# dsilvestro/npBNN

Hardware: AMD Instinct MI355X
Metric: MCMC iterations/sec (full fwd+lik per proposal) (higher is better)
Workload: dtype f16x3-split/f32

## Files before the change

### include/npbnn_hip.h

```cpp
#ifndef NPBNN_HIP_H
#define NPBNN_HIP_H

#include <stddef.h>
#include <stdint.h>

#ifdef __cplusplus
extern "C" {
#endif

#define NPBNN_ABI_VERSION 1
#define NPBNN_MAX_LAYERS 8
#define NPBNN_MAX_WIDTH 4096
#define NPBNN_MAX_TARGETS 16
#define NPBNN_XSTATE_DOUBLES (4 + NPBNN_MAX_TARGETS)

enum {
    NPBNN_OK = 0,
    NPBNN_E_ARG = -1,
    NPBNN_E_STATE = -2,
    NPBNN_E_HIP = -3,
    NPBNN_E_NOMEM = -4,
    NPBNN_E_COMM = -5,
    NPBNN_E_RANGE = -6,
    NPBNN_E_SYNC = -7,
// ... 130 lines not shown
    int32_t slope_term_in_prior;
} npbnn_chain_cfg;
#define NPBNN_SCHED_AUTO 0
#define NPBNN_SCHED_SERIAL 1
#define NPBNN_SCHED_OVERLAP 2
#define NPBNN_SCHED_OVERLAP2 3

#define NPBNN_SCHED_PERSIST 4

#define NPBNN_SCHED_PERSIST_SERIAL 5

typedef struct {
    double loglik, logprior;
    double sigma[NPBNN_MAX_TARGETS];
    int64_t n_accepted;
    int32_t n_passes;
    int32_t n_candidates;
    int32_t n_void_passes;
    int32_t schedule;
    double temperature;
    int32_t iterations_done;
    int32_t overflow;
    double slopes[NPBNN_MAX_LAYERS];
} npbnn_chain_result;

int npbnn_chain_run(npbnn_ctx* ctx, const npbnn_chain_cfg* cfg, double* W_inout, const double* mask_packed,
                    int32_t K, int32_t M, const int32_t* idx, const double* delta, const int32_t* cnt,
                    const double* log_u, uint8_t* out_accepted, double* out_loglik_prop, double* out_logprior_prop,
                    npbnn_chain_result* result);

enum { NPBNN_PROP_NORMAL = 0, NPBNN_PROP_UNIFORM = 1, NPBNN_PROP_FIXED_NORMAL = 2, NPBNN_PROP_NORMAL_NORMALIZED = 3 };
typedef struct {
    int32_t proposal_kind;
    int32_t M;
    const int32_t* idx;
    const double* val;
    const int32_t* cnt;
    const int32_t* h_idx;
    const double* h_val;
    const double* h_fac;
    const int32_t* h_cnt;
    const int32_t* layer_mask;
    double* ind_inout;
    const int32_t* ind_ptr;
    const int32_t* ind_pos;
    double prior_ind1;
// ... 76 lines not shown
```

### npbnn_amd/_capi.py

```python
import ctypes as C
import os

import numpy as np

MAX_LAYERS = 8
MAX_WIDTH = 4096
MAX_TARGETS = 16
XSTATE_DOUBLES = 4 + MAX_TARGETS

ACT_RELU, ACT_LEAKY, ACT_SWISH, ACT_TANH = 0, 1, 2, 3
OUT_SOFTMAX, OUT_IDENTITY, OUT_SOFTPLUS_HALF = 0, 1, 2
(LIK_CATEGORICAL, LIK_GAUSS, LIK_GAUSS_PRED_SIGMA, LIK_POISSON, LIK_NEGBIN, LIK_NEGBIN2D,
 LIK_NEGBIN_BASE10, LIK_NONE) = range(8)
PRIOR_UNIFORM, PRIOR_NORMAL, PRIOR_CAUCHY, PRIOR_LAPLACE = 0, 1, 2, 3
TRAIN, TEST = 0, 1
OPT_L0_PRECISION = 1
OPT_FAST_TAILS = 2
OPT_PERSISTENT = 3
OPT_TRAINABLE_SLOPES = 4
OPT_WIDE = 5
L0_AUTO, L0_F32, L0_F16 = 0, 1, 2
INFO_L0_F16, INFO_WAVES_PER_BLOCK, INFO_N_CU, INFO_FAST_TAILS, INFO_TURN_NS_OVERLAPPED, INFO_TURN_NS_BETWEEN, INFO_MAX_CANDIDATES = 1, 2, 3, 4, 5, 6, 7
INFO_IT_NS_OVERLAPPED, INFO_IT_NS_BETWEEN = 8, 9
INFO_WIDE = 10
# ... 32 lines not shown


class EvalOut(C.Structure):
    _fields_ = [("loglik", C.c_double), ("sigma", C.c_double * MAX_TARGETS),
                ("sum_r", C.c_double * MAX_TARGETS), ("sum_r2", C.c_double * MAX_TARGETS),
                ("n_rows", C.c_int64)]


class ChainCfg(C.Structure):
    _fields_ = [("prior_kind", C.c_int32), ("prior_scale", C.c_double * MAX_LAYERS), ("w_bound", C.c_double),
                ("temperature", C.c_double), ("lik_temp", C.c_double), ("sigma_given", C.c_int32),
                ("sigma", C.c_double * MAX_TARGETS), ("cur_loglik", C.c_double), ("cur_logprior", C.c_double),
                ("cur_sigma", C.c_double * MAX_TARGETS), ("force_f32", C.c_int32), ("n_candidates", C.c_int32),
                ("schedule", C.c_int32), ("reserved_", C.c_int32), ("sigma_mult", C.POINTER(C.c_double)),
                ("hastings", C.POINTER(C.c_double)), ("prior_scale_w", C.POINTER(C.c_double)),
                ("slope_idx", C.POINTER(C.c_int32)), ("slope_delta", C.POINTER(C.c_double)),
                ("cur_slopes", C.c_double * MAX_LAYERS), ("n_slopes", C.c_int32), ("slope_term_in_prior", C.c_int32)]


class ChainResult(C.Structure):
    _fields_ = [("loglik", C.c_double), ("logprior", C.c_double), ("sigma", C.c_double * MAX_TARGETS),
                ("n_accepted", C.c_int64), ("n_passes", C.c_int32), ("n_candidates", C.c_int32),
                ("n_void_passes", C.c_int32), ("schedule", C.c_int32), ("temperature", C.c_double),
                ("iterations_done", C.c_int32), ("overflow", C.c_int32), ("slopes", C.c_double * MAX_LAYERS)]


class GeneralCfg(C.Structure):
    _fields_ = [("proposal_kind", C.c_int32), ("M", C.c_int32), ("idx", C.POINTER(C.c_int32)), ("val", C.POINTER(C.c_double)),
                ("cnt", C.POINTER(C.c_int32)), ("h_idx", C.POINTER(C.c_int32)), ("h_val", C.POINTER(C.c_double)),
                ("h_fac", C.POINTER(C.c_double)), ("h_cnt", C.POINTER(C.c_int32)), ("layer_mask", C.POINTER(C.c_int32)),
                ("ind_inout", C.POINTER(C.c_double)), ("ind_ptr", C.POINTER(C.c_int32)), ("ind_pos", C.POINTER(C.c_int32)),
                ("prior_ind1", C.c_double), ("has_indicator_prior", C.c_int32), ("reserved_", C.c_int32),
                ("find_inout", C.POINTER(C.c_double)), ("feature_means", C.POINTER(C.c_double)),
                ("find_ptr", C.POINTER(C.c_int32)), ("find_pos", C.POINTER(C.c_int32)), ("find_use", C.POINTER(C.c_int32))]


PROP_NORMAL, PROP_UNIFORM, PROP_FIXED_NORMAL, PROP_NORMAL_NORMALIZED = 0, 1, 2, 3


class ChainJob(C.Structure):
    _fields_ = [("ctx", C.c_void_p), ("cfg", C.POINTER(ChainCfg)), ("W_inout", C.POINTER(C.c_double)),
                ("mask_packed", C.POINTER(C.c_double)), ("M", C.c_int32), ("chain_id", C.c_int32),
                ("idx", C.POINTER(C.c_int32)), ("delta", C.POINTER(C.c_double)), ("cnt", C.POINTER(C.c_int32)),
                ("log_u", C.POINTER(C.c_double)), ("out_accepted", C.POINTER(C.c_uint8)),
                ("out_loglik_prop", C.POINTER(C.c_double)), ("out_logprior_prop", C.POINTER(C.c_double)),
                ("out_state", C.POINTER(C.c_double)), ("out_cold_w", C.POINTER(C.c_double)),
                ("result", C.POINTER(ChainResult))]
# ... 125 lines not shown
```

### npbnn_amd/backend.py

```python
import ctypes as C
import os
from operator import is_ as _is
from time import perf_counter as _now

import numpy as np

from . import _capi as capi


_PACKED_VIEWS = {}


def note_packed_views(layers, base):
    if len(_PACKED_VIEWS) >= 32:
        _PACKED_VIEWS.clear()
    _PACKED_VIEWS[id(layers[0])] = (tuple(layers), base)


def pack_weights(weights):
    first = weights[0]
    known = _PACKED_VIEWS.get(id(first))
    if known is not None and len(known[0]) == len(weights) and all(map(_is, known[0], weights)):
        return known[1].copy()
    base = getattr(first, "base", None)
# ... 444 lines not shown
        k = self.arch.n_targets
        if sigma is not None:
            for j, v in enumerate(np.broadcast_to(sigma, (k,))):
                cfg.sigma[j] = float(v)
        if cur_sigma is not None:
            for j, v in enumerate(np.broadcast_to(cur_sigma, (k,))):
                cfg.cur_sigma[j] = float(v)
        cfg.cur_loglik, cfg.cur_logprior = float(cur_loglik), float(cur_logprior)
        cfg.n_candidates = int(n_candidates)
        cfg.schedule = int(schedule)
        cfg.force_f32 = 0
        if sigma_mult is not None:
            cfg._keep = (capi.as_f64(sigma_mult), capi.as_f64(hastings))
            cfg.sigma_mult, cfg.hastings = capi.dptr(cfg._keep[0]), capi.dptr(cfg._keep[1])
        else:
            cfg._keep = None
            cfg.sigma_mult = cfg.hastings = None

    def _result_dict(self, res):
        k = self.arch.n_targets
        return dict(loglik=res.loglik, logprior=res.logprior, sigma=np.array(res.sigma[:k]) if k else _NO_SIGMA,
                    n_accepted=res.n_accepted, n_passes=res.n_passes, n_candidates=res.n_candidates,
                    n_void_passes=res.n_void_passes, schedule=res.schedule, temperature=res.temperature,
                    iterations_done=res.iterations_done, overflow=res.overflow, slopes=res.slopes)

    def chain_run(self, weights, idx, delta, cnt, log_u, prior_kind, prior_scale, w_bound, temperature, lik_temp,
                  cur_loglik, cur_logprior, cur_sigma=None, sigma=None, mask=None, n_candidates=0, schedule=0, sigma_mult=None,
                  hastings=None, slopes=None, fixed_slopes=None):
        w = pack_weights(weights) if isinstance(weights, (list, tuple)) else capi.as_f64(weights).copy()
        K, M = idx.shape
        cfg = self.__dict__.get("_chain_cfg")
        if cfg is None:
            cfg = self._chain_cfg = capi.ChainCfg()
            self._chain_res = capi.ChainResult()
        self._fill_chain_cfg(cfg, prior_kind, prior_scale, w_bound, temperature, lik_temp, cur_loglik, cur_logprior,
                             cur_sigma, sigma, n_candidates, schedule, sigma_mult, hastings, slopes, fixed_slopes)
        m = None if mask is None else (pack_weights(mask) if isinstance(mask, (list, tuple)) else capi.as_f64(mask))
        if idx.dtype != np.int32 or not idx.flags.c_contiguous:
            idx = np.ascontiguousarray(idx, dtype=np.int32)
        if cnt.dtype != np.int32 or not cnt.flags.c_contiguous:
            cnt = np.ascontiguousarray(cnt, dtype=np.int32)
        delta = capi.as_f64(delta)
        log_u = capi.as_f64(log_u)
        acc = np.empty(K, dtype=np.uint8)
        llp, lpp = np.empty(K), np.empty(K)
        res = self._chain_res
        run = capi.chain_run_by_address(self._lib)
# ... 219 lines not shown
```

### npbnn_amd/csrc/npbnn_chain.hip.h

```cpp
#pragma once
#include "npbnn_common.hip.h"
#include "npbnn_pack.hip.h"

namespace npbnn {

struct FinalizeParams {
    const double* partials;
    int n_waves;
    int lik_kind;
    int k_targets;
    long long n_rows;
    double lik_temp;
    int sigma_given;
    double sigma[NPBNN_MAX_TARGETS];
    npbnn_eval_out* out;
};

__device__ __forceinline__ int partial_value_count(int lik_kind, int k_targets) { return lik_kind == NPBNN_LIK_GAUSS ? 1 + 2 * k_targets : 1; }
__device__ __forceinline__ int partial_value_index(int item, int k_targets) {
    return item <= k_targets ? item : 1 + NPBNN_MAX_TARGETS + (item - k_targets - 1);
}

__device__ __forceinline__ void reduce_partials(const double* __restrict__ partials, int n_blocks, int n_items, int k_targets, double* tot ) {
    const int lane = threadIdx.x & 63, wave = threadIdx.x >> 6, nw = blockDim.x >> 6;
// ... 39 lines not shown
    if (threadIdx.x == 0) loglik_from_totals(tot, f.lik_kind, f.k_targets, f.n_rows, f.lik_temp, f.sigma_given, f.sigma, f.out);
}
#endif

struct ChainDev {
    double logLik, logPrior;
    double sigma[NPBNN_MAX_TARGETS];
    double cand_logPrior[2][kMaxCand];
    int t;
    int n_accepted;
    int n_passes;
    int void_launch;
    int n_void;
    int seg_end;
    double temperature;
    double logPrior_rep;
    int seg_idx;
    int poisoned;
    int prepared;
    int aborted;
    int started;
    int exchanged;
    int done[4];
};

struct SlopeState {
    double cur[kMaxLayers];
    double term;
    double cand[2][kMaxCand][kMaxLayers];
};
__host__ __device__ inline double slope_prior_term(const double* s, int n) {
    double sum = 0.0;
    for (int l = 0; l < n; ++l) sum += s[l];
    return 2.302585092994046 * -sum * 10.0;
}

struct SpecState;
struct ChainParams {
    ChainDev* st;
    PassDesc* pass;
    double* w_cur;
    const double* mask;
    const int* idx;
    const double* delta;
    const int* cnt;
    const double* log_u;
// ... 146 lines not shown
    int out;
    int launch;
};
__device__ __forceinline__ StepPlan overlapped_plan(int launch) {
    StepPlan pl;
    pl.first = 0;
    pl.resum = 0;
    pl.dec = launch >= 1 ? ((launch - 1) & 1) : -1;
    pl.fly = launch & 1;
    pl.out = (launch + 1) & 1;
    pl.launch = launch;
    return pl;
}

struct StepShared {
    double tot[kMaxCand][kPartialStride];
    double red[16];
    double red3[kMaxCand][16];
    npbnn_eval_out o;
    double s_lp;
    int s_accepted, s_t, s_start, s_lim;
};

template <bool WIDE = false>
__device__ __forceinline__ void chain_step(const ChainParams& c_generic, const StepPlan pl, StepShared& sh) {
    typedef const __attribute__((address_space(4))) ChainParams ConstChainParams;
    ConstChainParams& c = *(ConstChainParams*)&c_generic;
    const int tid = threadIdx.x;
    ChainDev* st = c.st;
    const int lik_kind = c.net.lik_kind;
    const size_t pv_stride = (size_t)kMaxCand * c.M;
    const size_t part_stride = (size_t)kMaxCand * kPartialStride * c.n_blocks;
    const int stamp_row = pl.first ? 0 : (c.pass[pl.dec >= 0 ? pl.dec : 0].t0 & 1023);
#define NPBNN_STAMP(k) do { if (c.stamps && threadIdx.x == 0) c.stamps[(size_t)stamp_row * 8 + (k)] = wall_clock64(); } while (0)
    NPBNN_STAMP(0);

    if (pl.resum && c.prior_kind != NPBNN_PRIOR_UNIFORM) {
        double lp = 0.0;
        for (int l = 0; l < c.net.n_layers; ++l) {
            const auto& L = c.net.L[l];
            const int n = L.out_dim * (L.in_dim + L.has_bias);
            const double sc = c.prior_scale[l];
            if (c.prior_scale_w) {
                for (int i = tid; i < n; i += blockDim.x) lp += log_prior_density(c.prior_kind, c.w_cur[L.w_off + i], c.prior_scale_w[L.w_off + i]);
            } else if (c.prior_kind == NPBNN_PRIOR_NORMAL) {
                double q = 0.0;
                for (int i = tid; i < n; i += blockDim.x) { const double w = c.w_cur[L.w_off + i]; q += w * w; }
                lp += -0.5 * q / (sc * sc);
                if (tid == 0) lp -= (double)n * (log(sc) + 0.9189385332046727418);
            } else {
                for (int i = tid; i < n; i += blockDim.x) lp += log_prior_density(c.prior_kind, c.w_cur[L.w_off + i], sc);
            }
        }
        const double s = block_sum(lp, sh.red);
        if (tid == 0) st->logPrior = s;
    }
    if (pl.resum && c.slopes && tid == 0) {
        const double term = c.slope_term_in ? slope_prior_term(c.slopes->cur, c.n_slopes) : 0.0;
        c.slopes->term = term;
        if (c.prior_kind != NPBNN_PRIOR_UNIFORM) st->logPrior += term;
    }

    int t0 = 0, n_pend = 0;
    if (pl.dec >= 0) {
        t0 = c.pass[pl.dec].t0;
        n_pend = c.pass[pl.dec].n_cand;
        if (pl.fly >= 0 && st->void_launch == pl.launch - 1) n_pend = 0;
    }
    double prefetch_sink = 0.0;
    bool deferred = false;
    if constexpr (WIDE) deferred = c.prep_terms != nullptr;
    if (pl.fly < 0 && !deferred) {
        const int r_lo = t0 + (pl.first ? 0 : 1), r_hi = min(c.K, t0 + n_pend + c.D);
        double sink = 0.0;
        for (int r = r_lo; r < r_hi; ++r)
            if (tid < c.M) sink += (double)c.idx[(size_t)r * c.M + tid] + c.delta[(size_t)r * c.M + tid] + (double)c.pos[(size_t)r * c.M + tid];
        prefetch_sink = sink;
    }
    double d_cand[kMaxCand], d_logu[kMaxCand], d_h[kMaxCand], d_ll = 0.0, d_lp = 0.0, d_temp = 1.0;
#pragma unroll
    for (int j = 0; j < kMaxCand; ++j) { d_cand[j] = 0.0; d_logu[j] = 0.0; d_h[j] = 0.0; }
    if constexpr (WIDE) {
        if (deferred && n_pend > 0) {
            constexpr int TS = 3;
            int n_terms[kMaxCand];
            double x[kMaxCand][TS];
#pragma unroll
            for (int j = 0; j < kMaxCand; ++j) {
                n_terms[j] = j < n_pend ? c.pass[pl.dec].cnt[j] : 0;
#pragma unroll
// ... 57 lines not shown
                for (int b = lane + 256; b < c.n_blocks; b += 64) s += src[b];
                s = butterfly_sum_f64(s);
                if (lane == 0) sh.tot[j][v] = s;
            }
        }
        __syncthreads();
        NPBNN_STAMP(2);
        if (tid == 0) {
            int accepted = -1, n_done = n_pend;
#pragma unroll
            for (int j = 0; j < kMaxCand; ++j) {
                if (j < n_pend && accepted < 0) {
                    const int t = t0 + j;
                    if (c.sigma_mult) {
                        double sg[NPBNN_MAX_TARGETS];
                        for (int q = 0; q < c.net.k_targets; ++q) sg[q] = st->sigma[q] * c.sigma_mult[(size_t)t * c.net.k_targets + q];
                        loglik_from_totals(sh.tot[j], lik_kind, c.net.k_targets, c.n_rows, c.lik_temp, 1, sg, &sh.o);
                    } else {
                        loglik_from_totals(sh.tot[j], lik_kind, c.net.k_targets, c.n_rows, c.lik_temp, c.sigma_given, c_generic.sigma_fixed, &sh.o);
                    }
                    const double lp = d_cand[j];
                    const double post_new = sh.o.loglik + lp, post_old = d_ll + d_lp;
                    const int a = ((post_new - post_old) * d_temp + d_h[j] >= d_logu[j]) ? 1 : 0;
                    c.out_acc[t] = (unsigned char)a;
                    c.out_ll[t] = sh.o.loglik;
                    c.out_lp[t] = lp;
                    if (a) {
                        st->logLik = sh.o.loglik;
                        st->logPrior = lp;
                        st->logPrior_rep = lp;
                        st->n_accepted += 1;
                        if (lik_kind == NPBNN_LIK_GAUSS)
                            for (int q = 0; q < c.net.k_targets; ++q) st->sigma[q] = sh.o.sigma[q];
                        if (c.slopes) {
                            for (int l = 0; l < c.n_slopes; ++l) c.slopes->cur[l] = c.slopes->cand[pl.dec][j][l];
                            c.slopes->term = slope_prior_term(c.slopes->cur, c.n_slopes);
                        }
                        accepted = j;
                        n_done = j + 1;
                        sh.s_lp = lp;
                    }
                }
            }
            if (accepted < 0) sh.s_lp = d_lp;
            st->t = t0 + n_done;
            st->n_passes += 1;
            sh.s_accepted = accepted;
            sh.s_t = t0 + n_done;
            int start = t0 + n_done;
            if (pl.fly >= 0) {
                if (accepted >= 0) {
                    __hip_atomic_store(&st->void_launch, pl.launch, __ATOMIC_RELAXED, __HIP_MEMORY_SCOPE_AGENT);
                    if (c.pass[pl.fly].n_cand > 0) st->n_void += 1;
                } else {
                    start = c.pass[pl.fly].t0 + c.pass[pl.fly].n_cand;
                }
            }
            sh.s_start = start;
            sh.s_lim = st->seg_end;
        }
        __syncthreads();
        NPBNN_STAMP(3);
        const int a = sh.s_accepted;
        if constexpr (WIDE) {
            constexpr int CU = 4;
            if (a >= 0) {
                const size_t row = (size_t)(t0 + a) * c.M;
                const int n = c.cnt[t0 + a];
                const double* pv = c.pv + (size_t)pl.dec * pv_stride;
                for (int e0 = tid; e0 < n; e0 += CU * (int)blockDim.x) {
                    int ci[CU], cp[CU];
                    double cv[CU];
                    float cs[CU];
    #pragma unroll
                    for (int u = 0; u < CU; ++u) {
// ... 55 lines not shown

    NPBNN_STAMP(4);
    const int t_new = sh.s_start;
    int n_new = sh.s_lim - t_new;
    if (n_new > c.D) n_new = c.D;
    if (n_new < 0) n_new = 0;
    if (n_new == 0) {
        if (tid == 0) {
            PassDesc d;
            d.t0 = t_new;
            d.n_cand = 0;
            for (int j = 0; j < kMaxCand; ++j) d.cnt[j] = 0;
            d.pad[0] = sh.s_t >= sh.s_lim ? 1 : 0;
            d.pad[1] = d.pad[2] = 0;
            c.pass[pl.out] = d;
        }
        return;
    }
    double dlp[kMaxCand];
    if constexpr (WIDE) {
#pragma unroll
        for (int j = 0; j < kMaxCand; ++j) dlp[j] = 0.0;
    }
    if (!deferred) {
        const double* __restrict__ wcur = c.w_cur;
        const double* __restrict__ mask = c.mask;
        double* __restrict__ pv_out = c.pv + (size_t)pl.out * pv_stride;
        int woff[kMaxLayers];
        double half_inv_s2[kMaxLayers], layer_scale[kMaxLayers];
#pragma unroll
        for (int q = 0; q < kMaxLayers; ++q) {
            woff[q] = q < c.net.n_layers ? c.net.L[q].w_off : 0x7fffffff;
            half_inv_s2[q] = c.half_inv_s2[q];
            layer_scale[q] = c.prior_scale[q];
        }
        constexpr int ES = 2;
        int ii[kMaxCand][ES], pp[kMaxCand][ES], cn[kMaxCand];
        double dd[kMaxCand][ES], bb[kMaxCand][ES], mm[kMaxCand][ES], sw[kMaxCand][ES];
        float ss[kMaxCand][ES];
#pragma unroll
        for (int j = 0; j < kMaxCand; ++j) {
            dlp[j] = 0.0;
            cn[j] = j < n_new ? c.cnt[t_new + j] : 0;
#pragma unroll
            for (int u = 0; u < ES; ++u) {
                const int e = tid + u * (int)blockDim.x;
                ii[j][u] = -1; pp[j][u] = 0; dd[j][u] = 0.0; ss[j][u] = 1.0f;
                if (j < n_new && e < c.M) {
                    const size_t k = (size_t)(t_new + j) * c.M + e;
                    ii[j][u] = c.idx[k];
                    dd[j][u] = c.delta[k];
                    pp[j][u] = c.pos[k];
                    if (c.pscale) ss[j][u] = c.pscale[k];
                }
            }
        }
#pragma unroll
        for (int j = 0; j < kMaxCand; ++j)
#pragma unroll
            for (int u = 0; u < ES; ++u)
                if (!(tid + u * (int)blockDim.x < cn[j])) { ii[j][u] = -1; pp[j][u] = 0; dd[j][u] = 0.0; ss[j][u] = 1.0f; }
#pragma unroll
        for (int j = 0; j < kMaxCand; ++j)
#pragma unroll
            for (int u = 0; u < ES; ++u) {
                const int i = ii[j][u];
// ... 76 lines not shown
        PassDesc d;
        d.t0 = t_new;
        d.n_cand = n_new;
        for (int j = 0; j < kMaxCand; ++j) {
            double sj = 0.0;
            for (int w = 0; w < (int)(blockDim.x >> 6); ++w) sj += sh.red3[j][w];
            if (c.slopes && j < n_new) {
                const int k = c.slope_idx[t_new + j];
                const double step = c.slope_delta[t_new + j];
                double sum = 0.0;
                for (int l = 0; l < kMaxLayers; ++l) {
                    double v = l < c.n_slopes ? c.slopes->cur[l] : 0.0;
                    if (l == k) {
                        v += step;
                        if (v > 1.0) v = 1.0 - (v - 1.0);
                        if (v < 0.0) v = 0.0 + (0.0 - v);
                    }
                    c.slopes->cand[pl.out][j][l] = v;
                    if (l < c.n_slopes) sum += v;
                }
                sj += 2.302585092994046 * -sum * 10.0 - c.slopes->term;
            }
            if (j < n_new) st->cand_logPrior[pl.out][j] = base_lp + sj;
            d.cnt[j] = j < n_new ? c.cnt[t_new + j] : 0;
        }
        d.pad[0] = d.pad[1] = d.pad[2] = 0;
        c.pass[pl.out] = d;
    }
    if (prefetch_sink == 1.2345e300) c.out_lp[0] = prefetch_sink;
    NPBNN_STAMP(6);
#undef NPBNN_STAMP
}

constexpr unsigned long long kSyncTimeoutTicks = 25000000ull;

__device__ __forceinline__ bool sync_wait_ge(ChainDev* st, const int* word, int target, unsigned long long timeout_ticks = kSyncTimeoutTicks) {
    const unsigned long long t0 = wall_clock64();
    while (__hip_atomic_load(word, __ATOMIC_RELAXED, __HIP_MEMORY_SCOPE_AGENT) < target) {
        if (__hip_atomic_load(&st->aborted, __ATOMIC_RELAXED, __HIP_MEMORY_SCOPE_AGENT)) return false;
        if (wall_clock64() - t0 > timeout_ticks) {
            __hip_atomic_store(&st->aborted, 1, __ATOMIC_RELAXED, __HIP_MEMORY_SCOPE_AGENT);
            return false;
        }
        __builtin_amdgcn_s_sleep(2);
    }
    return !__hip_atomic_load(&st->aborted, __ATOMIC_RELAXED, __HIP_MEMORY_SCOPE_AGENT);
}
// ... 631 lines not shown
```

### npbnn_amd/csrc/npbnn_chain_api.hip

```cpp
#define NPBNN_KERNELS_CHAIN
#include "npbnn_ctx.hip.h"

extern "C" int npbnn_comm_allgather_inplace_stream_(npbnn_comm* c, double* d_buf, int count, void* stream);
extern "C" int npbnn_comm_info_(const npbnn_comm* c, int* device, int* rank, int* nranks);
extern "C" void npbnn_comm_abort_(npbnn_comm* c);
extern "C" int npbnn_comm_wait_stream_(npbnn_comm* c, void* stream, const char* what);

namespace {

struct ResLayout { size_t w, cnt, logu, acc, llp, lpp, total; };
ResLayout res_layout(size_t kc, size_t wb) {
    const auto up256 = [](size_t v) { return (v + 255) / 256 * 256; };
    ResLayout L;
    L.w = 512;
    L.cnt = L.w + up256(wb);
    L.logu = L.cnt + up256(kc * sizeof(int));
    L.acc = L.logu + up256(kc * sizeof(double));
    L.llp = L.acc + up256(kc);
    L.lpp = L.llp + up256(kc * sizeof(double));
    L.total = L.lpp + up256(kc * sizeof(double));
    return L;
}

struct ChainBatch {
// ... 215 lines not shown
        HIP_TRY(ctx, hipMemcpyAsync(ctx->d_delta, delta, need * sizeof(double), hipMemcpyHostToDevice, st));
    }
    stage_mark(ctx, "copy of indices + deviates", &t_stage);
    const bool f16 = ctx->net.l0_f16 != 0;
    ChainDev init{};
    init.logLik = cfg->cur_loglik;
    init.logPrior = cfg->cur_logprior;
    init.logPrior_rep = cfg->cur_logprior;
    for (int j = 0; j < NPBNN_MAX_TARGETS; ++j) init.sigma[j] = cfg->cur_sigma[j];
    init.t = 0;
    init.n_accepted = 0;
    init.n_passes = 0;
    init.void_launch = -2;
    init.n_void = 0;
    init.seg_end = (seg_len > 0 && seg_len < K) ? seg_len : K;
    init.temperature = cfg->temperature;
    init.seg_idx = 0;
    init.poisoned = 0;
    init.prepared = -1;
    init.aborted = 0;
    init.started = -1;
    init.exchanged = 0;
    for (int i = 0; i < 4; ++i) init.done[i] = 0;
    {
        memset(ctx->h_res, 0, 512);
        memcpy(ctx->h_res, &init, sizeof(ChainDev));
        memcpy(ctx->h_res + RL.w, W_in, wb);
        memcpy(ctx->h_res + RL.cnt, cnt, (size_t)K * sizeof(int));
        memcpy(ctx->h_res + RL.logu, log_u, (size_t)K * sizeof(double));
        HIP_TRY(ctx, hipMemcpyAsync(ctx->d_res, ctx->h_res, RL.acc, hipMemcpyHostToDevice, st));
    }
    stage_mark(ctx, "copy of state + weights", &t_stage);
    for (int l = 0; l < kMaxLayers; ++l)
        ctx->net.act_prm[l] = (!cfg->slope_idx && l < cfg->n_slopes && l < NPBNN_MAX_LAYERS) ? (float)cfg->cur_slopes[l] : 0.f;
    ChainParams c{};
    c.st = ctx->d_chain;
    c.pass = reinterpret_cast<PassDesc*>(reinterpret_cast<char*>(ctx->d_eparams) + offsetof(EvalParams, pass_desc));
    c.w_cur = ctx->d_wcur;
    c.mask = mask_packed ? ctx->d_mask : nullptr;
    c.idx = ctx->d_idx;
    c.delta = ctx->d_delta;
    c.cnt = ctx->d_cnt;
    c.log_u = ctx->d_logu;
    c.hastings = nullptr;
    c.sigma_mult = nullptr;
    if (cfg->sigma_mult || cfg->hastings) {
// ... 284 lines not shown
    const int overflow = (ctx->net.l0_f16 && (flags & kFlagF16Range)) ? 1 : 0;
    if (overflow && !exchange_run)
        return fail(ctx, NPBNN_E_RANGE, "chain_run: a layer-0 weight left the fp16 range during this batch");
    {
        const char* b = ctx->h_res;
        memcpy(W_inout, b + B.RL.w, B.wb);
        memcpy(out_accepted, b + B.RL.acc, (size_t)k_take);
        if (out_loglik_prop) memcpy(out_loglik_prop, b + B.RL.llp, (size_t)k_take * sizeof(double));
        if (out_logprior_prop) memcpy(out_logprior_prop, b + B.RL.lpp, (size_t)k_take * sizeof(double));
    }
    for (int l = 0; l < NPBNN_MAX_LAYERS; ++l) result->slopes[l] = 0.0;
    if (ctx->batch_slopes) {
        SlopeState fs;
        HIP_TRY(ctx, hipMemcpy(&fs, ctx->d_slopes, sizeof(SlopeState), hipMemcpyDeviceToHost));
        for (int l = 0; l < kMaxLayers && l < NPBNN_MAX_LAYERS; ++l) result->slopes[l] = fs.cur[l];
    }
    result->loglik = fin.logLik;
    result->logprior = fin.n_accepted > 0 ? fin.logPrior_rep : cfg->cur_logprior;
    for (int j = 0; j < NPBNN_MAX_TARGETS; ++j) result->sigma[j] = fin.sigma[j];
    result->n_accepted = fin.n_accepted;
    result->n_passes = fin.n_passes;
    result->n_candidates = B.D;
    result->n_void_passes = fin.n_void;
    result->schedule = B.schedule;
    result->temperature = fin.temperature;
    result->iterations_done = k_take;
    result->overflow = overflow;
    return NPBNN_OK;
}

}

extern "C" {

int npbnn_chain_run(npbnn_ctx* ctx, const npbnn_chain_cfg* cfg, double* W_inout, const double* mask_packed, int32_t K, int32_t M,
                    const int32_t* idx, const double* delta, const int32_t* cnt, const double* log_u, uint8_t* out_accepted,
                    double* out_loglik_prop, double* out_logprior_prop, npbnn_chain_result* result) {
    if (!ctx) return fail(nullptr, NPBNN_E_ARG, "null ctx");
    if (!result || !out_accepted) return fail(ctx, NPBNN_E_ARG, "chain_run: bad arguments");
    static const bool timing = getenv("NPBNN_CHAIN_TIMING") != nullptr;
    ChainBatch B;
    int rc = chain_prepare(ctx, cfg, W_inout, mask_packed, K, M, idx, delta, cnt, log_u, 0, &B);
    if (rc) return rc;
    hipStream_t st = ctx->stream;
    int t_done = 0, n_rounds = 0;
    const ChainDev* now = reinterpret_cast<const ChainDev*>(ctx->h_res.get());
// ... 456 lines not shown
```

### npbnn_amd/csrc/npbnn_eval.hip.h

```cpp
#pragma once
#include "npbnn_common.hip.h"
#include "npbnn_chain.hip.h"

namespace npbnn {

typedef void (*eval_fn_t)(const EvalParams*, int, int);
constexpr int kLikCat = 0, kLikGauss = 1, kLikGen = 2;
__host__ __device__ inline int lik_class(int lik_kind) {
    return lik_needs_row_scratch(lik_kind) ? kLikGen : (lik_kind == NPBNN_LIK_GAUSS ? kLikGauss : kLikCat);
}

template <int LK>
struct TileAcc {
    double ll;
};
template <>
struct TileAcc<kLikGauss> {
    double s1[4], s2[4];
};
constexpr int kFastGaussTargets = 2;

__device__ __forceinline__ int uni(int v) { return __builtin_amdgcn_readfirstlane(v); }
__device__ __forceinline__ float uni(float v) { return __uint_as_float(__builtin_amdgcn_readfirstlane(__float_as_uint(v))); }
__device__ __forceinline__ long long uni(long long v) {
// ... 402 lines not shown
    const int GN = (CHAIN && D > 1) ? uni(p.group_n) : 0;
    const int G = (int)gridDim.x - (GN ? GN : chain ? 1 : 0);
    if (GN && bid >= G) {
        StepShared& sh = *reinterpret_cast<StepShared*>(smem);
        chain_step(*uni(p.group[bid - G].chain), overlapped_plan(launch0), sh);
        return;
    }
    const bool sync = chain && uni(p.sync_mode);
    const int ebid = sync ? bid - 1 : bid;
    const int share_rot = (CHAIN && sync && !GN) ? uni(p.share_rot) : 0;
    int lbid = ebid;
    for (int i = 0; i < launch0 && share_rot > 0; ++i) { lbid += share_rot; if (lbid >= G) lbid -= G; }
    if (chain && bid == (sync ? 0 : G)) {
        StepShared& sh = *reinterpret_cast<StepShared*>(smem);
        int* const lds_flag = reinterpret_cast<int*>(smem + sizeof(StepShared));
        if (SPEC && uni(p.sync_mode) == 3) {
            SpecShared& sp = *reinterpret_cast<SpecShared*>(smem + ((sizeof(StepShared) + 64 + 15) & ~(size_t)15));
            if (chain->mask) spec_rounds<true>(*chain, launch0, launch_end, G, sh, sp, lds_flag);
            else spec_rounds<false>(*chain, launch0, launch_end, G, sh, sp, lds_flag);
            return;
        }
        for (int launch = launch0; launch < launch_end; ++launch) {
            if (sync && !sync_step_enter(*chain, launch, G, lds_flag)) return;
            chain_step(*chain, overlapped_plan(launch), sh);
            if (sync) sync_step_leave(chain->st, launch + 1, next_enqueued && launch + 1 == launch_end);
            if (launch + 1 < launch_end) {
                __syncthreads();
                if (threadIdx.x == 0) {
                    const PassDesc& nx = chain->pass[overlapped_plan(launch).out];
                    *lds_flag = (nx.n_cand == 0 && nx.pad[0] == 1) ? 1 : 0;
                }
                __syncthreads();
                if (*lds_flag) return;
                __syncthreads();
            }
        }
        return;
    }
#ifdef NPBNN_EXP_PROLOGUE_STAMPS
    unsigned long long t_prev_pass0 = 0;
#endif
    constexpr bool LOOK = CHAIN && !SPEC;
    int ahead_t0 = -1;
    int ahead_cnt[D];
#pragma unroll
    for (int j = 0; j < D; ++j) ahead_cnt[j] = 0;
    for (int launch = launch0; launch < launch_end; ++launch, lbid = (lbid + share_rot >= G ? lbid + share_rot - G : lbid + share_rot)) {
// ... 632 lines not shown
                consume();
            }
            if (n_issue < KT0) {
                NPBNN_WAIT_VMCNT(0);
                for (int kt = n_issue; kt < KT0; kt += STEP) consume();
            }
            q += KT0;
        } else {
            for (int kt = 0; kt < KT0; kt += STEP, q += STEP) {
                if (pf_q < Q) {
                    if constexpr (F16) issue_pair();
                    else issue_next();
                }
                wait_younger(pf_q - q - STEP);
                consume();
            }
        }

        if (void_flag) void_seen = __hip_atomic_load(void_flag, __ATOMIC_RELAXED, __HIP_MEMORY_SCOPE_AGENT);
        run_tail(acc0, tseq, tile);
    }
    }
    __builtin_amdgcn_s_waitcnt(0x0f70);
    const int tid_tiles = tid;
    {
    int tid_epi = tid_tiles;
    if constexpr (NPBNN_LAUNDER_TID) {
        tid_epi = threadIdx.x;
        asm volatile("" : "+v"(tid_epi));
    }
    const int tid = tid_epi;
    const int lane = tid & 63;
    const int n = lane & 15, kq = lane >> 4;

    NPBNN_ESTAMP(4);
    if (stamps && lane == 0) stamps[(size_t)gridDim.x * 8 + (size_t)bid * 16 + wave] = wall_clock64();
    const bool look = LOOK && sync && n_loop > 1 && launch + 1 < launch_end && !GN && g_partials != nullptr;
    int* const look_words = reinterpret_cast<int*>(smem + D * IB + (size_t)wpb * uni(p.lay.wave_lds));
    if (g_partials || GN) {
#pragma unroll
        for (int j = 0; j < D; ++j) {
            if constexpr (LK == kLikGauss) {
#pragma unroll
                for (int i = 0; i < GI; ++i) {
                    A[j].s1[i] = row_sum_f64(A[j].s1[i]);
                    A[j].s2[i] = row_sum_f64(A[j].s2[i]);
// ... 17 lines not shown
        }
        double* wsum = reinterpret_cast<double*>(smem + D * IB);
#pragma unroll
        for (int j = 0; j < D; ++j) {
            double* ws = wsum + ((size_t)j * wpb + wave) * kPartialStride;
            if constexpr (LK == kLikGauss) {
                if (lane == 0) ws[0] = 0.0;
                if (n == 0) {
#pragma unroll
                    for (int i = 0; i < 4; ++i) {
                        ws[1 + 4 * kq + i] = i < GI ? A[j].s1[i < GI ? i : 0] : 0.0;
                        ws[1 + NPBNN_MAX_TARGETS + 4 * kq + i] = i < GI ? A[j].s2[i < GI ? i : 0] : 0.0;
                    }
                }
            } else {
                if (lane == 0) ws[0] = A[j].ll;
            }
        }
        if (look && wave == 0 && lane < 8)
            look_words[lane] = nx_ready ? nx_desc : 0;
        asm volatile("" :: "v"(nx_prepared), "v"(nx_desc));
        __syncthreads();
        constexpr int nvals = (LK == kLikGauss) ? kPartialStride : 1;
        for (int item = tid - ((int)blockDim.x - 64); item >= 0 && item < D * nvals; item += 64) {
            const int j = item / nvals, v = item % nvals;
            if constexpr (LK == kLikGauss) { if (v != 0 && ((v - 1) & (NPBNN_MAX_TARGETS - 1)) >= p_generic.net.k_targets) continue; }
            double s = 0.0;
            for (int w = 0; w < wpb; ++w) s += wsum[((size_t)j * wpb + w) * kPartialStride + v];
            double* const dst = GN ? p.group[j].partials + (((size_t)par * kMaxCand) * kPartialStride + v) * G + lbid
                                   : g_partials + (((size_t)par * kMaxCand + j) * kPartialStride + v) * G + lbid;
            if constexpr (SPEC) {
                if (early_copy) { spec_part_store(spec_part + spec_part_index(par, j, v, lbid), s, spec_gen0 + (unsigned)launch + 1u); continue; }
            }
            if (sync) __hip_atomic_store(dst, s, __ATOMIC_RELAXED, __HIP_MEMORY_SCOPE_AGENT);
            else *dst = s;
        }
    }
    NPBNN_ESTAMP(6);
    if (sync) {
        __syncthreads();
        if (threadIdx.x == blockDim.x - 64 && !(SPEC && early_copy)) sync_eval_leave(st_dev, launch);
        if constexpr (LOOK) {
            if (look && look_words[1] > 0) {
                ahead_t0 = uni(look_words[0]);
#pragma unroll
                for (int j = 0; j < D; ++j) ahead_cnt[j] = uni(look_words[2 + (j < kMaxCand ? j : 0)]);
                stage_images();
            }
        }
    }
    }
    NPBNN_ESTAMPX(4);
    }
#undef NPBNN_ESTAMP
}

}
```

### npbnn_amd/sampler.py

```python
import _thread
import functools
import operator
import os
import queue
import threading

import numpy as np

from . import _capi as capi
from .backend import note_packed_views, pack_weights
from .likelihoods import (CalcAccuracy, CalcAccuracyRegression, CalcLabelAccuracy,
                          CalcLabelAccuracyRegression, SkipAccuracy, SkipAccuracyVec, calc_likelihood,
                          calc_likelihood_regression, calc_likelihood_regression_error, likelihood_kind,
                          stat_kind, stats_from_confusion)
from .model import data_transform_obj, npBNN
from .proposals import (UpdateBinomial, UpdateFixedNormal, UpdateNormal, UpdateNormal1D, UpdateNormalNormalized,
                        multiplier_proposal_vector)

_LAZY = ("_y", "_y_test", "_accuracy", "_test_accuracy", "_label_acc", "_label_freq")
_GENERAL_PROPOSALS = {UpdateNormal: capi.PROP_NORMAL, UpdateFixedNormal: capi.PROP_FIXED_NORMAL,
                      UpdateNormalNormalized: capi.PROP_NORMAL_NORMALIZED}

_POOL = None

# ... 206 lines not shown
                mcmc._speculation2 = second
                mcmc._cancel_second()
            ahead = self._draw_ahead(mcmc, it + k)
            fresh.append(ahead[1])
        further = self._draw_ahead(mcmc, it + 2 * k)
        fresh.append(further[1])
        try:
            rc = batch.run(w, idx, delta, cnt, log_u, mcmc._logLik, mcmc._logPrior, mcmc._temperature, cur_sigma, functools.partial(_enqueue_draws, fresh))
        finally:
            if ahead[1].queued:
                mcmc._speculation = ahead
                if further[1].queued:
                    mcmc._speculation2 = further
        if rc != 0:
            mcmc._cancel_speculation()
            done = _DrawJob(None)
            done.value = (idx, delta, cnt, log_u, None, None)
            done.done.release()
            mcmc._speculation = ((it, k) + self.key_tail, done, False, self.ws_src)
            return False
        res = batch.res
        sigma = np.array(res.sigma[:self.n_out]) if self.regression else None
        mcmc._absorb(bnn, k, w, batch.acc, int(res.n_accepted), res.n_passes, res.n_void_passes, res.schedule, res.loglik, res.logprior, sigma)
        self.layers = bnn._w_layers
        return True


class _Candidate:
    __slots__ = ("layers", "weight_switches", "feature_switches", "override", "sigma", "slopes_moved", "log_hastings",
                 "log_prior_extra", "log_prior", "log_lik", "log_post")

    def __init__(self, bnn_obj, log_prior_extra):
        self.layers = []
        self.weight_switches = bnn_obj._indicators + 0
        self.feature_switches = None
        self.override = None
        self.sigma = bnn_obj._error_prm
        self.slopes_moved = False
        self.log_hastings = 0
        self.log_prior_extra = log_prior_extra
        self.log_prior = self.log_lik = self.log_post = None


class MCMC():
    def __init__(self,
                 bnn_obj: npBNN,
# ... 559 lines not shown
            return
        try:
            spec[1].result()
        finally:
            if spec[2] and spec[1].saved is not None:
                self._gen.bit_generator.state = spec[1].saved

    @property
    def _rs(self):
        self._cancel_speculation()
        return self._gen

    @_rs.setter
    def _rs(self, value):
        self._cancel_speculation()
        self._gen = value

    n_candidates = 0
    device_schedule = 0
    _device_schedule_used = 0
    _device_accepted = 0
    _device_passes = 0
    _device_void_passes = 0
    _device_iterations = 0
    SUB_BATCH = 128
    SUB_BATCH_MAX = 512

    def _sub_batches(self, seg):
        sizes, k = [], self.SUB_BATCH
        while seg > 0:
            n = min(k, seg)
            sizes.append(n)
            seg -= n
            k = min(2 * k, self.SUB_BATCH_MAX)
        return sizes

    _slope_term_in_prior = False

    def _device_chain_cfg(self, bnn_obj, sigma_mult=None, hastings=None, slope_draws=None):
        regression = bnn_obj._estimation_mode == "regression"
        sigma = None
        cur_sigma = None
        if regression:
            cur_sigma = np.ones(bnn_obj._size_output) * bnn_obj._error_prm
            if not bnn_obj._empirical_error and sigma_mult is None:
                sigma = np.ones(bnn_obj._size_output)
# ... 13 lines not shown
        self._absorb_device_batch(bnn_obj, len(cnt), w_new, acc, res)
        if slope_draws is not None:
            act = bnn_obj._act_fun
            if res["n_accepted"] > 0:
                act.reset_prm(np.array(res["slopes"][:len(act._acc_prm)], dtype=float))
                act.reset_accepted_prm()
                self._slope_term_in_prior = True
            last = np.array(act._acc_prm, dtype=float)
            if not acc[len(cnt) - 1]:
                k = int(slope_draws[0][len(cnt) - 1])
                v = last[k] + slope_draws[1][len(cnt) - 1]
                if v > 1:
                    v = 1 - (v - 1)
                if v < 0:
                    v = 0 + (0 - v)
                last[k] = v
            act.reset_prm(last)

    def _absorb_device_batch(self, bnn_obj, k, w_new, acc, res):
        if k <= 0:
            return
        self._absorb(bnn_obj, k, w_new, acc, int(res.get("n_accepted", 0)), res.get("n_passes", k), res.get("n_void_passes", 0),
                     res.get("schedule", 0), res["loglik"], res["logprior"], res.get("sigma"))

    def _absorb(self, bnn_obj, k, w_new, acc, n_accepted, n_passes, n_void, schedule, loglik, logprior, sigma):
        acc = acc[:k]
        self._device_schedule_used = schedule
        self._device_accepted += n_accepted
        self._device_passes += n_passes
        self._device_void_passes += n_void
        self._device_iterations += k
        if n_accepted > 0:
            layers, off = [], 0
            for w in bnn_obj._w_layers:
                layers.append(w_new[off:off + w.size].reshape(w.shape))
                off += w.size
            if off == w_new.size and w_new.dtype == np.float64:
                note_packed_views(layers, w_new)
            bnn_obj.reset_weights(layers)
            self._logLik, self._logPrior = loglik, logprior
            self._logPost = self._logLik + self._logPrior
            if bnn_obj._estimation_mode == "regression":
                bnn_obj.reset_error_prm(sigma)
            self._accepted_override = None
            self._invalidate()
        history = self._last_accepted_mem + acc.tolist()
# ... 159 lines not shown
```

Baseline: 102,900.

## Signal void speculative passes early so eval skips their likelihood reduction

In the fast non-speculative overlapped chain path, the acceptance decision now publishes void_launch as soon as a candidate is accepted, instead of after the decision loop. The eval kernel checks this flag and skips the final likelihood partial reduction for a pass already known to be void, recording that it left early. The aim is to cut wasted likelihood work on speculative passes that an accepted proposal makes obsolete. It adds more cross-block atomic signalling and a new result counter, and the earlier flag publication could race with consumers that read it.

```diff
diff --git a/include/npbnn_hip.h b/include/npbnn_hip.h
--- a/include/npbnn_hip.h
+++ b/include/npbnn_hip.h
@@ -176,6 +176,8 @@
     int32_t iterations_done;
     int32_t overflow;
     double slopes[NPBNN_MAX_LAYERS];
+    int32_t n_void_left_early;
+    int32_t reserved_;
 } npbnn_chain_result;
 
 int npbnn_chain_run(npbnn_ctx* ctx, const npbnn_chain_cfg* cfg, double* W_inout, const double* mask_packed,
diff --git a/npbnn_amd/_capi.py b/npbnn_amd/_capi.py
--- a/npbnn_amd/_capi.py
+++ b/npbnn_amd/_capi.py
@@ -78,7 +78,8 @@
     _fields_ = [("loglik", C.c_double), ("logprior", C.c_double), ("sigma", C.c_double * MAX_TARGETS),
                 ("n_accepted", C.c_int64), ("n_passes", C.c_int32), ("n_candidates", C.c_int32),
                 ("n_void_passes", C.c_int32), ("schedule", C.c_int32), ("temperature", C.c_double),
-                ("iterations_done", C.c_int32), ("overflow", C.c_int32), ("slopes", C.c_double * MAX_LAYERS)]
+                ("iterations_done", C.c_int32), ("overflow", C.c_int32), ("slopes", C.c_double * MAX_LAYERS),
+                ("n_void_left_early", C.c_int32), ("reserved_", C.c_int32)]
 
 
 class GeneralCfg(C.Structure):
diff --git a/npbnn_amd/backend.py b/npbnn_amd/backend.py
--- a/npbnn_amd/backend.py
+++ b/npbnn_amd/backend.py
@@ -490,7 +490,8 @@
         return dict(loglik=res.loglik, logprior=res.logprior, sigma=np.array(res.sigma[:k]) if k else _NO_SIGMA,
                     n_accepted=res.n_accepted, n_passes=res.n_passes, n_candidates=res.n_candidates,
                     n_void_passes=res.n_void_passes, schedule=res.schedule, temperature=res.temperature,
-                    iterations_done=res.iterations_done, overflow=res.overflow, slopes=res.slopes)
+                    iterations_done=res.iterations_done, overflow=res.overflow, slopes=res.slopes,
+                    n_void_left_early=res.n_void_left_early)
 
     def chain_run(self, weights, idx, delta, cnt, log_u, prior_kind, prior_scale, w_bound, temperature, lik_temp,
                   cur_loglik, cur_logprior, cur_sigma=None, sigma=None, mask=None, n_candidates=0, schedule=0, sigma_mult=None,
diff --git a/npbnn_amd/csrc/npbnn_chain.hip.h b/npbnn_amd/csrc/npbnn_chain.hip.h
--- a/npbnn_amd/csrc/npbnn_chain.hip.h
+++ b/npbnn_amd/csrc/npbnn_chain.hip.h
@@ -85,6 +85,8 @@
     int started;
     int exchanged;
     int done[4];
+    int void_left;
+    int n_void_left;
 };
 
 struct SlopeState {
@@ -277,7 +279,7 @@
     int s_accepted, s_t, s_start, s_lim;
 };
 
-template <bool WIDE = false>
+template <bool WIDE = false, bool EXIT = false>
 __device__ __forceinline__ void chain_step(const ChainParams& c_generic, const StepPlan pl, StepShared& sh) {
     typedef const __attribute__((address_space(4))) ChainParams ConstChainParams;
     ConstChainParams& c = *(ConstChainParams*)&c_generic;
@@ -320,7 +322,12 @@
     if (pl.dec >= 0) {
         t0 = c.pass[pl.dec].t0;
         n_pend = c.pass[pl.dec].n_cand;
-        if (pl.fly >= 0 && st->void_launch == pl.launch - 1) n_pend = 0;
+        if (pl.fly >= 0 && st->void_launch == pl.launch - 1) {
+            n_pend = 0;
+            if constexpr (EXIT) {
+                if (tid == 0 && __hip_atomic_load(&st->void_left, __ATOMIC_RELAXED, __HIP_MEMORY_SCOPE_AGENT) == pl.launch - 1) st->n_void_left += 1;
+            }
+        }
     }
     double prefetch_sink = 0.0;
     bool deferred = false;
@@ -424,6 +431,9 @@
                     const double lp = d_cand[j];
                     const double post_new = sh.o.loglik + lp, post_old = d_ll + d_lp;
                     const int a = ((post_new - post_old) * d_temp + d_h[j] >= d_logu[j]) ? 1 : 0;
+                    if constexpr (EXIT) {
+                        if (a && pl.fly >= 0) __hip_atomic_store(&st->void_launch, pl.launch, __ATOMIC_RELAXED, __HIP_MEMORY_SCOPE_AGENT);
+                    }
                     c.out_acc[t] = (unsigned char)a;
                     c.out_ll[t] = sh.o.loglik;
                     c.out_lp[t] = lp;
@@ -452,7 +462,7 @@
             int start = t0 + n_done;
             if (pl.fly >= 0) {
                 if (accepted >= 0) {
-                    __hip_atomic_store(&st->void_launch, pl.launch, __ATOMIC_RELAXED, __HIP_MEMORY_SCOPE_AGENT);
+                    if constexpr (!EXIT) __hip_atomic_store(&st->void_launch, pl.launch, __ATOMIC_RELAXED, __HIP_MEMORY_SCOPE_AGENT);
                     if (c.pass[pl.fly].n_cand > 0) st->n_void += 1;
                 } else {
                     start = c.pass[pl.fly].t0 + c.pass[pl.fly].n_cand;
@@ -554,6 +564,9 @@
 #pragma unroll
         for (int j = 0; j < kMaxCand; ++j) dlp[j] = 0.0;
     }
+    int cnt_new[kMaxCand];
+#pragma unroll
+    for (int j = 0; j < kMaxCand; ++j) cnt_new[j] = -1;
     if (!deferred) {
         const double* __restrict__ wcur = c.w_cur;
         const double* __restrict__ mask = c.mask;
@@ -574,6 +587,7 @@
         for (int j = 0; j < kMaxCand; ++j) {
             dlp[j] = 0.0;
             cn[j] = j < n_new ? c.cnt[t_new + j] : 0;
+            if constexpr (EXIT) cnt_new[j] = cn[j];
 #pragma unroll
             for (int u = 0; u < ES; ++u) {
                 const int e = tid + u * (int)blockDim.x;
@@ -696,7 +710,7 @@
                 sj += 2.302585092994046 * -sum * 10.0 - c.slopes->term;
             }
             if (j < n_new) st->cand_logPrior[pl.out][j] = base_lp + sj;
-            d.cnt[j] = j < n_new ? c.cnt[t_new + j] : 0;
+            d.cnt[j] = j < n_new ? (cnt_new[j] >= 0 ? cnt_new[j] : c.cnt[t_new + j]) : 0;
         }
         d.pad[0] = d.pad[1] = d.pad[2] = 0;
         c.pass[pl.out] = d;
diff --git a/npbnn_amd/csrc/npbnn_chain_api.hip b/npbnn_amd/csrc/npbnn_chain_api.hip
--- a/npbnn_amd/csrc/npbnn_chain_api.hip
+++ b/npbnn_amd/csrc/npbnn_chain_api.hip
@@ -261,6 +261,8 @@
     init.started = -1;
     init.exchanged = 0;
     for (int i = 0; i < 4; ++i) init.done[i] = 0;
+    init.void_left = -2;
+    init.n_void_left = 0;
     {
         memset(ctx->h_res, 0, 512);
         memcpy(ctx->h_res, &init, sizeof(ChainDev));
@@ -591,6 +593,8 @@
     result->n_passes = fin.n_passes;
     result->n_candidates = B.D;
     result->n_void_passes = fin.n_void;
+    result->n_void_left_early = fin.n_void_left;
+    result->reserved_ = 0;
     result->schedule = B.schedule;
     result->temperature = fin.temperature;
     result->iterations_done = k_take;
diff --git a/npbnn_amd/csrc/npbnn_eval.hip.h b/npbnn_amd/csrc/npbnn_eval.hip.h
--- a/npbnn_amd/csrc/npbnn_eval.hip.h
+++ b/npbnn_amd/csrc/npbnn_eval.hip.h
@@ -448,7 +448,7 @@
         }
         for (int launch = launch0; launch < launch_end; ++launch) {
             if (sync && !sync_step_enter(*chain, launch, G, lds_flag)) return;
-            chain_step(*chain, overlapped_plan(launch), sh);
+            chain_step<false, FAST && !SPEC>(*chain, overlapped_plan(launch), sh);
             if (sync) sync_step_leave(chain->st, launch + 1, next_enqueued && launch + 1 == launch_end);
             if (launch + 1 < launch_end) {
                 __syncthreads();
@@ -1127,6 +1127,7 @@
     }
     }
     __builtin_amdgcn_s_waitcnt(0x0f70);
+    const bool pass_void = CHAIN && FAST && !SPEC && void_flag && uni(void_seen) == launch;
     const int tid_tiles = tid;
     {
     int tid_epi = tid_tiles;
@@ -1190,7 +1191,7 @@
         asm volatile("" :: "v"(nx_prepared), "v"(nx_desc));
         __syncthreads();
         constexpr int nvals = (LK == kLikGauss) ? kPartialStride : 1;
-        for (int item = tid - ((int)blockDim.x - 64); item >= 0 && item < D * nvals; item += 64) {
+        for (int item = tid - ((int)blockDim.x - 64); item >= 0 && item < D * nvals && !pass_void; item += 64) {
             const int j = item / nvals, v = item % nvals;
             if constexpr (LK == kLikGauss) { if (v != 0 && ((v - 1) & (NPBNN_MAX_TARGETS - 1)) >= p_generic.net.k_targets) continue; }
             double s = 0.0;
@@ -1204,6 +1205,10 @@
             else *dst = s;
         }
     }
+    if constexpr (CHAIN) {
+        if (pass_void && ebid == 0 && threadIdx.x == blockDim.x - 64)
+            __hip_atomic_store(&st_dev->void_left, launch, __ATOMIC_RELAXED, __HIP_MEMORY_SCOPE_AGENT);
+    }
     NPBNN_ESTAMP(6);
     if (sync) {
         __syncthreads();
diff --git a/npbnn_amd/sampler.py b/npbnn_amd/sampler.py
--- a/npbnn_amd/sampler.py
+++ b/npbnn_amd/sampler.py
@@ -252,6 +252,7 @@
         res = batch.res
         sigma = np.array(res.sigma[:self.n_out]) if self.regression else None
         mcmc._absorb(bnn, k, w, batch.acc, int(res.n_accepted), res.n_passes, res.n_void_passes, res.schedule, res.loglik, res.logprior, sigma)
+        mcmc._device_void_left_early += int(getattr(res, "n_void_left_early", 0))
         self.layers = bnn._w_layers
         return True
 
@@ -857,6 +858,7 @@
     _device_accepted = 0
     _device_passes = 0
     _device_void_passes = 0
+    _device_void_left_early = 0
     _device_iterations = 0
     SUB_BATCH = 128
     SUB_BATCH_MAX = 512
@@ -916,6 +918,7 @@
             return
         self._absorb(bnn_obj, k, w_new, acc, int(res.get("n_accepted", 0)), res.get("n_passes", k), res.get("n_void_passes", 0),
                      res.get("schedule", 0), res["loglik"], res["logprior"], res.get("sigma"))
+        self._device_void_left_early += int(res.get("n_void_left_early", 0))
 
     def _absorb(self, bnn_obj, k, w_new, acc, n_accepted, n_passes, n_void, schedule, loglik, logprior, sigma):
         acc = acc[:k]
```

Result: no change. 102,100 (-0.8%).
